# mfkiwl/erlangnetwork-gnsslib-sdr

Measured on AMD Instinct MI355X. Metric: correlations/sec (1 ms coh) + x real-time, 32-SV L1CA @16.368 Msps, higher is better.
Workload: dtype int8 samples x int8 carrier LUT -> int32 accumulators (exact); NCOs: the reference's fp64 running sums, bit for bit; 1 GPU; BASELINE configs[2]: 32-SV GPS L1CA tracking, 5-tap E/P/L correlators (CORRN=2, CORRD=3), 1 ms coherent, 16.368 Msps int8 IQ, per GPU; channels_per_gpu=32, epochs_per_launch=1000, taps=5, loop=open (frequencies held per launch); see closed_loop (--full), if_broadcast=none (1 GPU)

## Files before the change

erlangnetwork-gnsslib-sdr_amd/csrc/gnsscorr_nco.h:

```cpp
#pragma once

#include <math.h>
#include <stdint.h>
#include <string.h>
#include <type_traits>

#if defined(__HIPCC__)
#define GC_HD __host__ __device__ inline
#define GC_HDM __host__ __device__
#define GC_HD_NOINLINE __host__ __device__ __attribute__((noinline))
#else
#define GC_HD static inline
#define GC_HDM
#define GC_HD_NOINLINE static
#endif
#if defined(__clang__)
#define GC_FP_STRICT _Pragma("clang fp contract(off)")
#else
#define GC_FP_STRICT
#endif

#if defined(__HIP_DEVICE_COMPILE__)
#define GC_DDIV(a, b) __ddiv_rn((a), (b))
#else
// ... 1488 lines not shown
    GC_FP_STRICT
    if (C.ex0 == GC_NO_TABLE || n < 1) return false;
    double x = gc_div_y(remcarr * GC_NCO_CDIV, GC_NCO_DPI, P.ydpi);
    if (!gc_one_binade_walk(x, C.s, n, &x)) return false;
    bool held;
    const double p = gc_prem_checked(x, kprem, &held);
    if (!held) return false;
    *remcarr_out = p;
    return true;
}

#define GC_REC_TAG(c)    ((c) & 3)
#define GC_REC_NMATCH    (1 << 2)
#define GC_REC_WALK      (1 << 3)
#define GC_REC_P0(c)     (((c) >> 4) & 15)
#define GC_REC_PLAST(c)  (((c) >> 8) & 15)
#define GC_REC_KPREM(c)  (((c) >> 12) & 15)
#define GC_REC_TIE       (1 << 16)
#define GC_REC_ONE       (1 << 17)
#define GC_REC_ROW1      (1 << 18)
struct GcCarRec {
    double lo, hi;
    double dmd[GC_CLAIM_CWIN];
    int ctl;
    int key;
};

GC_HD bool gc_one_binade_consts(int ex, double s, double *d, bool *tie, double *top)
{
    GC_FP_STRICT
    const uint64_t us = gc_d2u(s);
    const int es = gc_expo(s);
    *tie = false;
    if (ex == 0 || ex == 0x7FF || es == 0 || es == 0x7FF) return false;
    const int et = es + 1075 - ex;
    if (et >= 1023 + 51) return false;
    double b = 0.0;
    if (et >= 1023 - 1) {
        const double t = gc_u2d((us & 0x800FFFFFFFFFFFFFull) | ((uint64_t)et << 52));
        b = rint(t);
        *tie = fabs(t - b) == 0.5;
    }
    *d = ldexp(b, ex - 1075);
    *top = gc_u2d(((uint64_t)ex << 52) | 0x000FFFFFFFFFFFFFull);
    return true;
}

GC_HD void gc_car_rec_make(GcCarRec &R, const GcCarClaims &row, int n, int ilo, int ex0, double s, double ydpi)
{
    GC_FP_STRICT
    int tag = row.tag & 3;
    const int p0 = row.i0 - ilo, plast = p0 + row.nseg - 1;
    if (tag == 1 && !(p0 >= 0 && plast >= p0 && plast < GC_CLAIM_CWIN)) tag = 3;
    if ((tag == 1 || tag == 2) && !(row.kprem >= 0 && row.kprem <= GC_CLAIM_PREM)) tag = 3;
    int ctl = tag | ((row.tag & 3) == 1 ? GC_REC_ROW1 : 0);
    ctl |= n == row.nl ? GC_REC_NMATCH : 0;
    ctl |= (n > 0 && n <= (1 << 24)) ? GC_REC_WALK : 0;
    R.lo = row.lo;
    R.hi = row.hi;
    R.key = 0;
    for (int p = 0; p < GC_CLAIM_CWIN; p++) R.dmd[p] = 0.0;
    if (tag == 1) {
        ctl |= (p0 << 4) | (plast << 8) | (row.kprem << 12);
        for (int p = 0; p < GC_CLAIM_CWIN; p++) R.dmd[p] = (double)row.dm[p];
    } else if (tag == 2) {
        ctl |= row.kprem << 12;
        const double xlo = gc_div_y(row.lo * GC_NCO_CDIV, GC_NCO_DPI, ydpi);
        const double xhi = gc_div_y(row.hi * GC_NCO_CDIV, GC_NCO_DPI, ydpi);
        const int klo = (int)(gc_d2u(xlo) >> 52), khi = (int)(gc_d2u(xhi) >> 52);
        double d, top;
        bool tie;
        if (ex0 != GC_NO_TABLE && klo == khi && (klo >> 11) == (int)(gc_d2u(s) >> 63) &&
            gc_one_binade_consts(klo & 0x7FF, s, &d, &tie, &top)) {
            ctl |= GC_REC_ONE | (tie ? GC_REC_TIE : 0);
            R.key = klo;
            R.dmd[0] = d;
            R.dmd[1] = top;
            R.dmd[2] = (double)n;
        }
    }
    R.ctl = ctl;
}

GC_HD bool gc_carrier_rec_step_one(double ydpi, double remcarr, int key, bool tie, double d, double top, double nd, int kprem,
                                   double *remcarr_out)
{
    GC_FP_STRICT
    const double x = gc_div_y(remcarr * GC_NCO_CDIV, GC_NCO_DPI, ydpi);
    const uint64_t ux = gc_d2u(x);
    if ((int)(ux >> 52) != key) return false;
    if (tie && (ux & 1)) return false;
    const double y = fma(nd, d, x);
    if (!(fabs(y) <= top)) return false;
    bool held;
    const double p = gc_prem_checked(y, kprem, &held);
    if (!held) return false;
    *remcarr_out = p;
    return true;
}

struct GcCodeScanRow {
    long long Yhat, K;
    double r1;
    int valid, pad;
};

GC_HD double gc_code_scan_head(double remcode, double smaxci, double dlen, bool *neg, int *ecs)
{
    GC_FP_STRICT
    const double cs = remcode - smaxci;
    *neg = cs < 0.0;
    *ecs = gc_expo(cs);
    return cs + dlen;
}

GC_HD double gc_code_scan_u(double dlen) { return gc_u2d((uint64_t)(gc_expo(gc_u2d(gc_d2u(dlen) - 1)) - 52) << 52); }
GC_HD double gc_code_scan_invu(double dlen) { return gc_u2d((uint64_t)(2046 - (gc_expo(gc_u2d(gc_d2u(dlen) - 1)) - 52)) << 52); }

GC_HD void gc_code_scan_row(GcCodeScanRow &R, const GcCodePlan &P, double lo, double hi, double r1lo, double r1hi)
{
    GC_FP_STRICT
    R.Yhat = R.K = 0;
    R.r1 = r1lo;
    R.valid = R.pad = 0;
    if (!P.ok || P.it >= P.itop) return;
    const int etop = gc_expo(P.limtop);
    bool n0, n1, n2, n3;
    int e0, e1, e2, e3;
    const double y0 = gc_code_scan_head(lo, P.smaxci, P.dlen, &n0, &e0), y1 = gc_code_scan_head(hi, P.smaxci, P.dlen, &n1, &e1);
    const double z0 = gc_code_scan_head(r1lo, P.smaxci, P.dlen, &n2, &e2), z1 = gc_code_scan_head(r1hi, P.smaxci, P.dlen, &n3, &e3);
    if (!(n0 && n1 && n2 && n3) || e0 != e1 || e2 != e3) return;
    if (gc_expo(y0) != etop || gc_expo(y1) != etop || gc_expo(z0) != etop || gc_expo(z1) != etop) return;
    if (!(y0 < P.dlen && y1 < P.dlen && z0 < P.dlen && z1 < P.dlen)) return;
    const double invu = gc_code_scan_invu(P.dlen);
    const double k0 = (z0 - y0) * invu, k1 = (z1 - y1) * invu;
    if (!(k0 == k1) || !(fabs(k0) < 4503599627370496.0) || floor(k0) != k0) return;
    R.Yhat = (long long)(y0 * invu);
    R.K = (long long)k0;
    R.valid = 1;
}

GC_HD double gc_code_scan_next(double r1, long long Yhat, long long Y, double u)
{
    GC_FP_STRICT
    return r1 + (double)(Y - Yhat) * u;
}
```

erlangnetwork-gnsslib-sdr_amd/csrc/gnsscorr_plan.hip:

```cpp
#include <cstdlib>
#include <cstddef>
#include <hip/hip_runtime.h>

#include "gnsscorr_internal.h"

namespace {


#define GC_SPEC_WC  9.313225746154785e-10
#define GC_SPEC_WK  9.313225746154785e-10

struct SpecChan {
    GcCodePlan PC;
    GcCarPlan PK;
    GcCarStepC CK;
    double ci, spc, ps, dlen;
    int clen, smax;
    int tmax;
    bool ok;
};

__device__ __forceinline__ void spec_chan_init(SpecChan &C, const GcChan &c, const GcTrkState &s, bool with_prem)
{
    C.ci = __dmul_rn(c.ti, s.codefreq);
// ... 102 lines not shown
    srow.r1 = 0.0;
    srow.valid = srow.pad = 0;
    if (C.ok) {
        double r0, g0;
        int nhat;
        gc_spec_start(s.remcode, s.remcarr, C.ci, C.spc, C.ps, C.dlen, e, &r0, &g0, &nhat);
        const double rt = r0 + sumc, gt = g0 + sumk;
        int ncode = 0;
        bool bracketed = false;
#pragma unroll 1
        for (int att = 0; att < 2 && !bracketed; att++) {
            const double w = att == 0 ? GC_SPEC_WC : GC_SPEC_WC * 0.00390625;
            const double lo = rt - w, hi = rt + w;
            const int nlo = gc_period_nsamp(C.dlen, lo, C.spc), nhi = gc_period_nsamp(C.dlen, hi, C.spc);
            if (!(nlo == nhi && nlo > 0 && nlo <= (1 << 24))) continue;
            double flo = 0.0, fhi = 0.0;
            const bool side = (lo - C.PC.smaxci < 0.0) == (hi - C.PC.smaxci < 0.0);
            const bool oklo = gc_code_claims<true>(C.PC, lo, nlo + 2 * C.smax, cc, &flo);
            const bool okhi = oklo && gc_code_claims<false>(C.PC, hi, nlo + 2 * C.smax, cc, &fhi);
            const bool tailfits = nlo + 2 * C.smax - cc.jsum <= C.tmax;
            if (side && oklo && okhi && tailfits) {
                bracketed = true;
                ncode = nlo;
                cc.tag = 1;
                cc.n = nlo;
                cc.lo = lo;
                cc.hi = hi;
                gc_code_scan_row(srow, C.PC, lo, hi, flo, fhi);
            }
        }
        if (!bracketed) {
            ncode = gc_period_nsamp(C.dlen, rt, C.spc);
            cc.tag = 0;
            if (ncode > 0 && ncode <= (1 << 24)) {
                double dummy;
                cc.tag = (gc_code_claims<true>(C.PC, rt, ncode + 2 * C.smax, cc, &dummy) && ncode + 2 * C.smax - cc.jsum <= C.tmax) ? 3 : 0;
            }
            cc.n = ncode;
            cc.lo = cc.hi = rt;
        }
        const int nk = ncode;
        if (nk > 0 && nk <= (1 << 24)) {
            bool kbr = false;
            int tag = 0;
#pragma unroll 1
            for (int att = 0; att < 2 && !kbr; att++) {
                const double w = fmax(GC_SPEC_WK, fabs(gt) * 1.4551915228366852e-11) * (att == 0 ? 1.0 : 0.00390625);
                const double klo = gt - w, khi = gt + w;
                double dummy;
                bool ok = gc_carrier_claims_step<true>(C.PK, C.CK, klo, nk, ck, &dummy);
                tag = ck.tag;
                ok = ok && gc_carrier_claims_step<false, true>(C.PK, C.CK, khi, nk, ck, &dummy);
                if (ok) {
                    kbr = true;
                    ck.tag = tag;
                    ck.lo = klo;
                    ck.hi = khi;
                }
            }
            if (!kbr) {
                double dummy;
                const bool ok = gc_carrier_claims_step<true>(C.PK, C.CK, gt, nk, ck, &dummy);
                ck.tag = ok ? (ck.tag == 2 ? 2 : 3) : 0;
                ck.lo = ck.hi = gt;
            }
            ck.nl = nk;
        }
    }
    const size_t row = (size_t)ch * nepoch + eb;
    int4 *rc = reinterpret_cast<int4 *>(claims_code) + row * (GC_CLAIM_ROW / 4);
    int4 *rk = reinterpret_cast<int4 *>(claims_car) + row * (GC_CLAIM_ROW / 4);
    const int4 *pc4 = reinterpret_cast<const int4 *>(&cc), *pk4 = reinterpret_cast<const int4 *>(&ck);
#pragma unroll
    for (int q = 0; q < GC_CLAIM_ROW / 4; q++) {
        rc[q] = pc4[q];
        rk[q] = pk4[q];
    }
    scan[row] = srow;
}

__device__ unsigned long long gc_plan_stats[8];
#define GC_PLAN_REC_CH 64
__device__ unsigned long long gc_plan_rec[2 * GC_PLAN_REC_CH];
__device__ unsigned long long gc_plan_scan[GC_PLAN_REC_CH];

__host__ __device__ inline int plan2_class(double ti, double codefreq, int clen, int smax)
{
    const double ci = ti * codefreq;
    if (!(ci > 0.0) || !gc_fast_has_table(ci)) return -1;
    const int itop = gc_expo(gc_u2d(gc_d2u((double)clen) - 1)) - (gc_expo(ci) + 2);
    if (itop < 7 || itop > 12) return -1;
    if (smax + 1 > GC_CLAIM_TAIL2) return -1;
    return (itop - 7) * 3 + gc_tail_class(smax);
}

#define GC_PLAN_MAXE 4096
__device__ __attribute__((noinline)) void trk_plan_body(const GcChan *__restrict__ chan,
                                                        const GcTrkState *__restrict__ state_in,
                                                        GcTrkState *__restrict__ state_out,
                                                        GcTrkPlan *__restrict__ plan, int nch, int nepoch)
{
    __shared__ int nsh[GC_PLAN_MAXE];
    __shared__ int prog;
    const int ch = blockIdx.x, lane = threadIdx.x & 63, wave = threadIdx.x >> 6;
    if (ch >= nch) return;
    __builtin_amdgcn_s_setprio(3);
    const bool split = nepoch <= GC_PLAN_MAXE;
    if (threadIdx.x == 0) prog = 0;
    __syncthreads();
    if (!split && wave == 1) return;
    const GcChan c = chan[ch];
    GcTrkState s = state_in[ch];
    const double ci = __dmul_rn(c.ti, s.codefreq);
    const double spc = __ddiv_rn(s.codefreq, c.f_sf);
    const double ps = gc_carrier_ps(s.carrfreq, c.ti);
    const double dlen = (double)c.clen;
    const bool code_ok = ci > 0.0 && ci < dlen;
    GcTrkPlan *out = plan + (size_t)ch * nepoch;
    GcNoEmit ne;
    GcFillLanes fill{lane};
    const bool do_code = wave == 0, do_car = wave == 1 || !split;
    GcCodePlan PC;
    GcCarPlan PK;
    if (do_code) gc_code_plan_init(PC, ci, c.clen, c.smax);
    if (do_car) gc_car_plan_init(PK, ps);
    const double yspc = gc_period_yspc(spc);
    unsigned tally[6] = {0, 0, 0, 0, 0, 0};
    for (int e = 0; e < nepoch; e++) {
        int n;
        if (do_code) {
            n = gc_period_nsamp(dlen, s.remcode, spc, yspc);
            if (lane == 0) {
                out[e].buffloc = s.buffloc;
                out[e].coff = s.remcode;
                out[e].carrfreq = s.carrfreq;
                out[e].codefreq = s.codefreq;
                out[e].n = n;
                out[e].pad = 0;
            }
            if (split) {
                if (lane == 0) nsh[e] = n;
                __threadfence_block();
                if (lane == 0) __hip_atomic_store(&prog, e + 1, __ATOMIC_RELEASE, __HIP_MEMORY_SCOPE_WORKGROUP);
            }
        } else {
            while (__hip_atomic_load(&prog, __ATOMIC_ACQUIRE, __HIP_MEMORY_SCOPE_WORKGROUP) <= e) __builtin_amdgcn_s_sleep(1);
            n = nsh[e];
        }
        const bool walk = n > 0 && n <= (1 << 24);
        if (do_car) {
            if (lane == 0) out[e].phi0 = s.remcarr;
            if (walk) {
                int tier;
                s.remcarr = gc_carrier_period_any(PK, s.remcarr, n, fill, ne, &tier);
                if (tier == GC_TIER_PERIOD) tally[4]++;
                else tally[5]++;
            }
        }
        if (do_code) {
            if (walk && code_ok) {
                int tier;
                s.remcode = gc_code_period_any(PC, s.remcode, n + 2 * c.smax, fill, ne, &tier);
                if (tier == GC_TIER_PERIOD) tally[1]++;
                else tally[2]++;
            }
            s.buffloc += (uint64_t)(int64_t)n;
// ... 30 lines not shown
    GcCarPlan pkfull;
};
__shared__ __attribute__((aligned(16))) Plan4Shared g_plan4;

__device__ __forceinline__ int plan2_uni(int v) { return __builtin_amdgcn_readfirstlane(v); }
template <class T>
__device__ __forceinline__ T *plan2_uni(T *p)
{
    const uint64_t u = (uint64_t)p;
    const unsigned lo = (unsigned)__builtin_amdgcn_readfirstlane((int)(unsigned)u);
    const unsigned hi = (unsigned)__builtin_amdgcn_readfirstlane((int)(unsigned)(u >> 32));
    return (T *)(((uint64_t)hi << 32) | lo);
}
__device__ __forceinline__ double plan2_uni(double x)
{
    const uint64_t u = gc_d2u(x);
    const unsigned lo = (unsigned)__builtin_amdgcn_readfirstlane((int)(unsigned)u);
    const unsigned hi = (unsigned)__builtin_amdgcn_readfirstlane((int)(unsigned)(u >> 32));
    return gc_u2d(((uint64_t)hi << 32) | lo);
}

#define GC_CONST __attribute__((address_space(4)))
typedef int gc_v4i __attribute__((ext_vector_type(4)));
__device__ __forceinline__ GcCodeClaims plan4_code_row(const GC_CONST gc_v4i *r)
{
    const gc_v4i v0 = r[0], v1 = r[1], v2 = r[2], v3 = r[3], v4 = r[4], v5 = r[5];
    GcCodeClaims c;
    c.tag = v0.x; c.i0 = v0.y; c.q = v0.z; c.nl = v0.w;
    c.jsum = v1.x; c.dm[0] = v1.y; c.dm[1] = v1.z; c.dm[2] = v1.w;
    c.dm[3] = v2.x; c.dm[4] = v2.y; c.dm[5] = v2.z; c.dm[6] = v2.w;
    c.dm[7] = v3.x; c.dm[8] = v3.y; c.dm[9] = v3.z; c.dm[10] = v3.w;
    c.dm[11] = v4.x; c.dm[12] = v4.y; c.n = v4.z; c.pad = 0;
    c.lo = gc_u2d(((uint64_t)(unsigned)v5.y << 32) | (unsigned)v5.x);
    c.hi = gc_u2d(((uint64_t)(unsigned)v5.w << 32) | (unsigned)v5.z);
    return c;
}
template <class RowPtr>
__device__ __forceinline__ GcCarClaims plan4_car_row(RowPtr r)
{
    const gc_v4i v0 = r[0], v1 = r[1], v2 = r[2], v3 = r[3], v5 = r[5];
    GcCarClaims c;
    c.tag = v0.x; c.nl = v0.y; c.i0 = v0.z; c.nseg = v0.w;
    c.kprem = v1.x; c.dm[0] = v1.y; c.dm[1] = v1.z; c.dm[2] = v1.w;
    c.dm[3] = v2.x; c.dm[4] = v2.y; c.dm[5] = v2.z; c.dm[6] = v2.w;
    c.dm[7] = v3.x; c.dm[8] = v3.y; c.dm[9] = v3.z; c.dm[10] = v3.w;
    c.dm[11] = 0; c.dm[12] = 0; c.pad[0] = 0; c.pad[1] = 0;
    c.lo = gc_u2d(((uint64_t)(unsigned)v5.y << 32) | (unsigned)v5.x);
    c.hi = gc_u2d(((uint64_t)(unsigned)v5.w << 32) | (unsigned)v5.z);
    return c;
}
static_assert(GC_CLAIM_CWIN <= 11, "plan4_car_row reads dm[0..10]");
static_assert(sizeof(GcCodeClaims) == GC_CLAIM_ROW * 4 && sizeof(GcCarClaims) == GC_CLAIM_ROW * 4, "claims rows are GC_CLAIM_ROW ints");
static_assert(offsetof(GcCodeClaims, dm) == 20 && offsetof(GcCarClaims, dm) == 20, "claims layout");
static_assert(offsetof(GcCodeClaims, n) == 72 && offsetof(GcCodeClaims, lo) == 80 && offsetof(GcCarClaims, lo) == 80, "claims layout");
static_assert(GC_CLAIM_ROW == 24, "plan4_*_row read six int4 per row");

__device__ __attribute__((noinline)) int plan2_code_slow(double ci_, int clen_, int smax_, double remcode_, int n_, int lane, double *out)
{
    const double ci = plan2_uni(ci_), remcode = plan2_uni(remcode_);
    const int clen = plan2_uni(clen_), smax = plan2_uni(smax_), n = plan2_uni(n_);
    GcCodePlan PC;
    gc_code_plan_init(PC, ci, clen, smax);
    GcFillLanes fill{lane};
    GcNoEmit ne;
    int tier;
    *out = gc_code_period_any(PC, remcode, n + 2 * smax, fill, ne, &tier);
    return tier == GC_TIER_PERIOD ? 1 : 2;
}

__device__ __attribute__((noinline)) int plan2_car_slow(double remcarr_, int n_, int lane, double *out)
{
    const double remcarr = plan2_uni(remcarr_);
    const int n = plan2_uni(n_);
    const GcCarPlan &PK = g_plan4.pkfull;
    GcFillLanes fill{lane};
    GcNoEmit ne;
    int tier;
    *out = gc_carrier_period_any(PK, remcarr, n, fill, ne, &tier);
    return tier == GC_TIER_PERIOD ? 1 : 2;
}

#ifdef GC_PLAN_PROF
__device__ unsigned long long gc_plan_prof[64 * 16];
#define GC_PP_DECL unsigned long long pp_[7] = {0, 0, 0, 0, 0, 0, 0}
#define GC_PP_T0(v) const unsigned long long v = __builtin_readcyclecounter()
#define GC_PP_ADD(k, v) pp_[k] += __builtin_readcyclecounter() - (v)
#define GC_PP_INC(k) pp_[k] += 1
#define GC_PP_ADDN(k, n) pp_[k] += (n)
#define GC_PP_OUT(which) do { if (lane == 0 && blockIdx.x < 64) for (int k_ = 0; k_ < 7; k_++) atomicAdd(&gc_plan_prof[blockIdx.x * 16 + (which) * 8 + k_], pp_[k_]); } while (0)
#else
#define GC_PP_DECL do { } while (0)
#define GC_PP_T0(v) do { } while (0)
#define GC_PP_ADD(k, v) do { } while (0)
#define GC_PP_INC(k) do { } while (0)
#define GC_PP_ADDN(k, n) do { } while (0)
#define GC_PP_OUT(which) do { } while (0)
#endif
struct Plan4Job {
    const int4 *claims_code, *claims_car;
    const GcCodeScanRow *scan;
    GcTrkPlan *out;
    GcTrkState *state_out;
    GcTrkState s;
    int nepoch, nblk, verify;
};

__device__ __forceinline__ Plan4Job plan4_job(const Plan4Job *J_)
{
    Plan4Job J = *plan2_uni(J_);
    J.claims_code = plan2_uni(J.claims_code);
    J.claims_car = plan2_uni(J.claims_car);
    J.scan = plan2_uni(J.scan);
    J.out = plan2_uni(J.out);
    J.state_out = plan2_uni(J.state_out);
    J.nepoch = plan2_uni(J.nepoch);
    J.nblk = plan2_uni(J.nblk);
    J.verify = plan2_uni(J.verify);
    return J;
}

__device__ __forceinline__ int plan4_nb(const Plan4Job &J, int b)
{
    const int left = J.nepoch - b * GC_P4_BLK;
    return left < GC_P4_BLK ? left : GC_P4_BLK;
}

#define GC_GLOBAL __attribute__((address_space(1)))
__device__ __forceinline__ void plan4_publish(int v)
{
    asm volatile("" ::: "memory");
    __hip_atomic_store(&g_plan4.prog, v, __ATOMIC_RELAXED, __HIP_MEMORY_SCOPE_WORKGROUP);
}
__device__ __forceinline__ int plan4_progress()
{
    const int v = __hip_atomic_load(&g_plan4.prog, __ATOMIC_RELAXED, __HIP_MEMORY_SCOPE_WORKGROUP);
    asm volatile("" ::: "memory");
    return v;
}
template <int ITOP, int TMAX>
__device__ __attribute__((noinline)) int plan4_code_other(double ci_, int clen_, int smax_, double remcode_, int n_, int lane, const GcCodeClaims *cl_, double *out)
{
    const GcCodeClaims *clp = plan2_uni(cl_);
    if (plan2_uni(clp->tag) == 1 || plan2_uni(clp->tag) == 3) {
        const double ci = plan2_uni(ci_), remcode = plan2_uni(remcode_);
        const int clen = plan2_uni(clen_), smax = plan2_uni(smax_), n = plan2_uni(n_);
        GcCodePlan PC;
        gc_code_plan_init(PC, ci, clen, smax, false);
        GcCodeStepC<ITOP> SC;
        gc_code_stepc_init(SC, PC);
        GcCodeClaims c2 = *clp;
        c2.tag = 1;
        double rc;
        if (gc_code_claims_step<ITOP, TMAX, false, true>(PC, SC, remcode, n + 2 * smax, c2, &rc)) { *out = rc; return 0; }
    }
    return plan2_code_slow(ci_, clen_, smax_, remcode_, n_, lane, out);
}

__device__ __forceinline__ int plan4_scopy(int x)
{
    int c;
    asm volatile("s_mov_b32 %0, %1" : "=s"(c) : "s"(x));
    return c;
}
__device__ __forceinline__ bool plan4_bcopy(bool x) { return __builtin_amdgcn_readfirstlane(x ? 1 : 0) != 0; }

__device__ __forceinline__ long long plan4_wscan(long long v, int lane)
// ... 255 lines not shown
        const int n = plan2_uni(n_), nsamp = plan2_uni(nsamp_);
        GcCarPlan PK;
        gc_car_plan_init(PK, ps, false, false);
        GcCarStepC CK;
        gc_car_stepc_init(CK, PK, nsamp + 16);
        GcCarClaims c2 = *clp;
        c2.tag = tag == 2 ? 2 : 1;
        double rp;
        if (gc_carrier_claims_step<false, true>(PK, CK, remcarr, n, c2, &rp)) { *out = rp; return 0; }
    }
    return plan2_car_slow(remcarr_, n_, lane, out);
}

__device__ __attribute__((noinline)) void plan4_car_cert_wave(double ps_, const Plan4Job *J_, int lane)
{
    const double ps = plan2_uni(ps_);
    const Plan4Job J = plan4_job(J_);
    GcCarPlan PK;
    gc_car_plan_init(PK, ps);
    GcFillLanes fill{lane};
    GcNoEmit ne;
    unsigned tally1 = 0, tally2 = 0;
    GC_GLOBAL GcTrkPlan *out = (GC_GLOBAL GcTrkPlan *)J.out;
    double remcarr = J.s.remcarr;
    int seen = 0;
    for (int b = 0; b < J.nblk; b++) {
        const int nb = plan4_nb(J, b), e0 = b * GC_P4_BLK;
        for (int i = 0; i < nb; i++) {
            while (seen <= e0 + i) {
                seen = plan2_uni(plan4_progress());
                if (seen <= e0 + i) __builtin_amdgcn_s_sleep(1);
            }
            const int n = plan2_uni(g_plan4.nsh[e0 + i]);
            if (lane == 0) g_plan4.vstart[1][i] = remcarr;
            if (n > 0 && n <= (1 << 24)) {
                int tier;
                remcarr = gc_carrier_period_any(PK, remcarr, n, fill, ne, &tier);
                tally1 += tier == GC_TIER_PERIOD ? 1 : 0;
                tally2 += tier == GC_TIER_PERIOD ? 0 : 1;
            }
        }
        if (lane < nb) out[e0 + lane].phi0 = g_plan4.vstart[1][lane];
    }
    if (lane == 0) {
        ((GC_GLOBAL GcTrkState *)J.state_out)->remcarr = remcarr;
        if (tally1) atomicAdd(&gc_plan_stats[4], (unsigned long long)tally1);
        if (tally2) atomicAdd(&gc_plan_stats[5], (unsigned long long)tally2);
    }
}

__device__ __attribute__((noinline)) int plan4_car_one(double s_, int ex0_, double remcarr_, int n_, int ctl_, int key_, double d_, double top_,
                                                       double nd_, int verify_, double *out)
{
    const int verify = plan2_uni(verify_);
    const double s = plan2_uni(s_), remcarr = plan2_uni(remcarr_), d = plan2_uni(d_), top = plan2_uni(top_), nd = plan2_uni(nd_);
    const int ex0 = plan2_uni(ex0_), n = plan2_uni(n_), ctl = plan2_uni(ctl_), key = plan2_uni(key_);
    GcCarPlan P;
    P.ydpi = 1.0 / GC_NCO_DPI;
    GcCarStepC C;
    C.s = s;
    C.ex0 = ex0;
    double r = remcarr, r2 = remcarr;
    const bool done = gc_carrier_value_step_one(P, C, remcarr, n, GC_REC_KPREM(ctl), &r);
    int bad = 0;
    if (verify && (ctl & GC_REC_ONE)) {
        const bool done2 = gc_carrier_rec_step_one(P.ydpi, remcarr, key, (ctl & GC_REC_TIE) != 0, d, top, nd, GC_REC_KPREM(ctl), &r2);
        bad = (done2 && (!done || gc_d2u(r2) != gc_d2u(r))) ? 2 : 0;
    }
    if (done) *out = r;
    return (done ? 1 : 0) | bad;
}

__device__ __forceinline__ void plan4_rec_load(GcCarRec &R, int i)
{
    const GcCarRec &r = g_plan4.rec[i];
    R.lo = r.lo;
    R.hi = r.hi;
#pragma unroll
    for (int p = 0; p < GC_CLAIM_CWIN; p++) R.dmd[p] = r.dmd[p];
    R.ctl = r.ctl;
    R.key = r.key;
}

struct Plan4CarRun {
    double remcarr, phi;
    unsigned recwin, recone;
    unsigned tally0, tally1, tally2, miss, mism, slow;
    unsigned long long slowclk;
};

#ifdef GC_PLAN_PROF
#define GC_PP_SLOW0(v) const unsigned long long v = __builtin_readcyclecounter()
#define GC_PP_SLOW1(S, v) (S).slowclk += __builtin_readcyclecounter() - (v)
#else
#define GC_PP_SLOW0(v) do { } while (0)
#define GC_PP_SLOW1(S, v) do { } while (0)
#endif

__device__ __forceinline__ void plan4_car_period(Plan4CarRun &S, const GcCarRec &R, const GcCarPlan &PK, const GcCarStepC &CK, double ps, int nsamp,
                                                 const Plan4Job &J, int e, int i, int lane)
{
    const int ctl = plan2_uni(R.ctl);
    const int tag = GC_REC_TAG(ctl);
    const double remcarr = S.remcarr;
    const bool inside_u = plan4_bcopy(remcarr >= R.lo && remcarr <= R.hi) && (ctl & (3 | GC_REC_NMATCH)) == (1 | GC_REC_NMATCH);
    S.phi = lane == i ? remcarr : S.phi;
    if (!(ctl & GC_REC_WALK)) return;
    double rp = remcarr;
    bool done = false;
    if (inside_u && !J.verify) {
        rp = gc_carrier_value_step(PK, CK, remcarr, GC_REC_P0(ctl), GC_REC_PLAST(ctl), GC_REC_KPREM(ctl), R.dmd);
        done = true;
        S.recwin++;
    } else if (tag == 2) {
        if ((ctl & GC_REC_ONE) && !J.verify) {
            double r2 = remcarr;
            done = plan4_bcopy(gc_carrier_rec_step_one(PK.ydpi, remcarr, plan2_uni(R.key), (ctl & GC_REC_TIE) != 0, R.dmd[0], R.dmd[1], R.dmd[2],
                                                       GC_REC_KPREM(ctl), &r2));
            rp = done ? r2 : rp;
            S.recone += done ? 1 : 0;
        }
        if (!done) {
            double r1;
            const int n = plan2_uni(g_plan4.nsh[e]);
            GC_PP_SLOW0(pone_);
            const int how = plan4_car_one(CK.s, CK.ex0, remcarr, n, ctl, R.key, R.dmd[0], R.dmd[1], R.dmd[2], J.verify, &r1);
            GC_PP_SLOW1(S, pone_);
            done = (how & 1) != 0;
            S.slow++;
            S.tally0 += done ? 1 : 0;
            S.mism += (how & 2) ? 1 : 0;
            if (done) rp = r1;
        }
    }
    if (!done) {
        double rs;
        const int n = plan2_uni(g_plan4.nsh[e]);
        GC_PP_SLOW0(pother_);
        const int how = plan4_car_other(ps, nsamp, remcarr, n, lane, reinterpret_cast<const GcCarClaims *>(J.claims_car) + e, &rs);
        GC_PP_SLOW1(S, pother_);
        S.slow++;
        S.tally0 += how == 0 ? 1 : 0;
        S.tally1 += how == 1 ? 1 : 0;
        S.tally2 += how == 2 ? 1 : 0;
        S.mism += (inside_u && how != 0) ? 1 : 0;
        S.miss += (!inside_u && (ctl & GC_REC_ROW1)) ? 1 : 0;
        rp = rs;
    }
    S.remcarr = rp;
}

__device__ __attribute__((noinline)) void plan4_car_wave(double ps_, int nsamp_, const Plan4Job *J_, int lane)
{
    const int nsamp = plan2_uni(nsamp_);
    const double ps = plan2_uni(ps_);
    const Plan4Job J = plan4_job(J_);
    {
        const int nlook = J.nepoch < 16 ? J.nepoch : 16;
        int none = 0;
        for (int e = 0; e < nlook; e++)
            none += ((const GC_CONST int *)J.claims_car)[(size_t)e * GC_CLAIM_ROW] == 0 ? 1 : 0;
        if (none == nlook && nlook >= 8) {
            plan4_car_cert_wave(ps, J_, lane);
            return;
        }
    }
    {
        GcCarPlan full;
        gc_car_plan_init(full, ps);
        if (lane == 0) g_plan4.pkfull = full;
    }
    GcCarPlan PK;
    gc_car_plan_init(PK, ps, false, false);
    GcCarStepC CK;
    gc_car_stepc_init(CK, PK, nsamp + 16);
    const int ilo = plan2_uni(CK.ilo), ex0 = plan2_uni(CK.ex0);
    GC_GLOBAL GcTrkPlan *out = (GC_GLOBAL GcTrkPlan *)J.out;
    Plan4CarRun S;
    S.remcarr = J.s.remcarr;
    S.phi = 0.0;
    S.recwin = S.recone = S.tally0 = S.tally1 = S.tally2 = S.miss = S.mism = S.slow = 0;
    S.slowclk = 0;
    int seen = 0;
    GC_PP_DECL;
    GC_PP_T0(ptot_);
    for (int b = 0; b < J.nblk; b++) {
        const int nb = plan4_nb(J, b), e0 = b * GC_P4_BLK;
        GC_PP_T0(ptop_);
        const int el = e0 + (lane < nb ? lane : nb - 1);
        const GcCarClaims row = plan4_car_row((const GC_GLOBAL gc_v4i *)J.claims_car + (size_t)el * (GC_CLAIM_ROW / 4));
        if (seen < e0 + nb) {
            GC_PP_T0(pn_);
            while (seen < e0 + nb) {
                seen = plan2_uni(plan4_progress());
                if (seen < e0 + nb) __builtin_amdgcn_s_sleep(1);
            }
            GC_PP_ADD(3, pn_);
        }
        {
            GcCarRec mine;
            gc_car_rec_make(mine, row, g_plan4.nsh[el], ilo, ex0, CK.s, PK.ydpi);
            if (lane < nb) g_plan4.rec[lane] = mine;
        }
        asm volatile("" ::: "memory");
        __builtin_amdgcn_wave_barrier();
        GC_PP_ADD(5, ptop_);
        GC_PP_T0(pstep_);
        GcCarRec A, B;
        plan4_rec_load(A, 0);
        for (int i = 0; i < nb; i += 2) {
            plan4_rec_load(B, i + 1 < nb ? i + 1 : i);
            __builtin_amdgcn_sched_barrier(0);
            plan4_car_period(S, A, PK, CK, ps, nsamp, J, e0 + i, i, lane);
            if (i + 1 >= nb) break;
            plan4_rec_load(A, i + 2 < nb ? i + 2 : i + 1);
            __builtin_amdgcn_sched_barrier(0);
            plan4_car_period(S, B, PK, CK, ps, nsamp, J, e0 + i + 1, i + 1, lane);
        }
        GC_PP_ADD(6, pstep_);
        if (lane < nb) out[e0 + lane].phi0 = S.phi;
    }
    GC_PP_ADD(0, ptot_);
    GC_PP_ADDN(1, S.slowclk);
    GC_PP_ADDN(4, S.slow);
    GC_PP_OUT(1);
    if (lane == 0) {
        ((GC_GLOBAL GcTrkState *)J.state_out)->remcarr = S.remcarr;
        S.tally0 += S.recwin + S.recone;
        if (blockIdx.x < GC_PLAN_REC_CH) {
            if (S.recwin) atomicAdd(&gc_plan_rec[blockIdx.x * 2], (unsigned long long)S.recwin);
            if (S.recone) atomicAdd(&gc_plan_rec[blockIdx.x * 2 + 1], (unsigned long long)S.recone);
        }
        if (S.tally0) atomicAdd(&gc_plan_stats[3], (unsigned long long)S.tally0);
        if (S.tally1) atomicAdd(&gc_plan_stats[4], (unsigned long long)S.tally1);
        if (S.tally2) atomicAdd(&gc_plan_stats[5], (unsigned long long)S.tally2);
        if (S.mism) atomicAdd(&gc_plan_stats[6], (unsigned long long)S.mism);
        if (S.miss) atomicAdd(&gc_plan_stats[7], (unsigned long long)S.miss);
    }
}

template <int ITOP>
__device__ __forceinline__ void plan4_code_dispatch(int tcls, double ci, double spc, int clen, int smax, const Plan4Job *J, int lane)
{
    if (tcls == 0) plan4_code_wave<ITOP, gc_tail_max(0)>(ci, spc, clen, smax, J, lane);
    else if (tcls == 1) plan4_code_wave<ITOP, gc_tail_max(1)>(ci, spc, clen, smax, J, lane);
    else plan4_code_wave<ITOP, gc_tail_max(2)>(ci, spc, clen, smax, J, lane);
}

__global__ __launch_bounds__(128) void trk_plan4_kernel(const GcChan *__restrict__ chan, const GcTrkState *__restrict__ state_in,
                                                        GcTrkState *__restrict__ state_out, GcTrkPlan *__restrict__ plan,
                                                        int nch, int nepoch, const int *__restrict__ claims_code,
                                                        const int *__restrict__ claims_car, const GcCodeScanRow *__restrict__ scan, int verify)
{
    const int ch = blockIdx.x, tid = threadIdx.x, lane = tid & 63, wave = tid >> 6;
    if (ch >= nch) return;
    const GcChan c = chan[ch];
    const GcTrkState s = state_in[ch];
    const double ci = __dmul_rn(c.ti, s.codefreq), spc = __ddiv_rn(s.codefreq, c.f_sf), ps = gc_carrier_ps(s.carrfreq, c.ti);
    const int cls = plan2_class(c.ti, s.codefreq, c.clen, c.smax);
    if (cls < 0 || !(ci > 0.0 && ci < (double)c.clen)) {
        trk_plan_body(chan, state_in, state_out, plan, nch, nepoch);
        return;
    }
    const int itop = cls / 3 + 7, tcls = cls % 3;
    constexpr int RW4 = GC_CLAIM_ROW / 4;
    Plan4Job J;
    J.claims_code = reinterpret_cast<const int4 *>(claims_code) + (size_t)ch * nepoch * RW4;
    J.claims_car = reinterpret_cast<const int4 *>(claims_car) + (size_t)ch * nepoch * RW4;
    J.scan = scan ? scan + (size_t)ch * nepoch : nullptr;
    J.out = plan + (size_t)ch * nepoch;
    J.state_out = state_out + ch;
    J.s = s;
    J.nepoch = nepoch;
    J.nblk = (nepoch + GC_P4_BLK - 1) / GC_P4_BLK;
    J.verify = verify;
    if (tid == 0) g_plan4.prog = 0;
    __syncthreads();
    __builtin_amdgcn_s_setprio(3);
    if (wave == 0) {
        gc_with_itop(itop, [&](auto IT) { plan4_code_dispatch<decltype(IT)::value>(tcls, ci, spc, c.clen, c.smax, &J, lane); return true; });
    } else {
        plan4_car_wave(ps, c.nsamp, &J, lane);
    }
}


}


#ifdef GC_PLAN_PROF
extern "C" int gnsscorr_debug_plan_prof(unsigned long long *dst)
{
    if (hipMemcpyFromSymbol(dst, HIP_SYMBOL(gc_plan_prof), sizeof(unsigned long long) * 64 * 16) != hipSuccess) return -1;
    return 0;
}
#endif

extern "C" int gnsscorr_debug_plan_stats(unsigned long long *dst, int reset)
{
    if (hipMemcpyFromSymbol(dst, HIP_SYMBOL(gc_plan_stats), sizeof(unsigned long long) * 8) != hipSuccess) return -1;
    if (reset) {
        unsigned long long z[8] = {0, 0, 0, 0, 0, 0, 0, 0};
        if (hipMemcpyToSymbol(HIP_SYMBOL(gc_plan_stats), z, sizeof(z)) != hipSuccess) return -1;
    }
    return 0;
}

extern "C" int gnsscorr_debug_plan_rec(unsigned long long *dst, int reset)
{
    if (hipMemcpyFromSymbol(dst, HIP_SYMBOL(gc_plan_rec), sizeof(unsigned long long) * 2 * GC_PLAN_REC_CH) != hipSuccess) return -1;
    if (reset) {
        unsigned long long z[2 * GC_PLAN_REC_CH] = {0};
        if (hipMemcpyToSymbol(HIP_SYMBOL(gc_plan_rec), z, sizeof(z)) != hipSuccess) return -1;
    }
    return 0;
}

extern "C" int gnsscorr_debug_plan_scan(unsigned long long *dst, int reset)
{
    if (hipMemcpyFromSymbol(dst, HIP_SYMBOL(gc_plan_scan), sizeof(unsigned long long) * GC_PLAN_REC_CH) != hipSuccess) return -1;
    if (reset) {
        unsigned long long z[GC_PLAN_REC_CH] = {0};
        if (hipMemcpyToSymbol(HIP_SYMBOL(gc_plan_scan), z, sizeof(z)) != hipSuccess) return -1;
    }
    return 0;
}

static bool trk_nospec()
{
    static const bool nospec = getenv("GNSSCORR_TRK_NOSPEC") != nullptr;
    return nospec;
}

size_t gc_trk_spec_ints(size_t units) { return units * (2 * GC_CLAIM_ROW + 8 + 8); }
static_assert(sizeof(GcCodeScanRow) == 32 && ((2 * GC_CLAIM_ROW + 8) * 4) % 32 == 0, "scan rows lie 32-byte aligned behind the deviations");
static GcCodeScanRow *trk_scan_rows(int *claims, size_t units) { return reinterpret_cast<GcCodeScanRow *>(claims + units * (2 * GC_CLAIM_ROW + 8)); }

int gc_launch_trk_spec(hipStream_t st, const GcChan *chan, const GcTrkState *state_in, int nch, int nepoch, int *claims,
                       int e_off)
{
    if (!claims || trk_nospec() || nepoch > GC_PLAN_MAXE || e_off < 0 || e_off > nepoch) return 0;
    const size_t units = (size_t)nch * nepoch;
    const int T = e_off + nepoch;
    double *devc = reinterpret_cast<double *>(claims + 2 * units * GC_CLAIM_ROW), *devk = devc + 2 * units;
    hipLaunchKernelGGL(trk_specdev_kernel, dim3((nch * T + 63) / 64), dim3(64), 0, st, chan, state_in, devc, devk, nch, T);
    GC_HIP(hipGetLastError());
    const int nchunk = (nepoch + GC_SPEC_CHUNK - 1) / GC_SPEC_CHUNK;
    hipLaunchKernelGGL(trk_spec_kernel, dim3(nch * nchunk), dim3(GC_SPEC_CHUNK), 0, st, chan, state_in, devc, devk, claims,
                       claims + units * GC_CLAIM_ROW, trk_scan_rows(claims, units), nch, nepoch, e_off);
    GC_HIP(hipGetLastError());
    return 0;
}

int gc_launch_trk_plan(hipStream_t st, const GcChan *chan, const GcTrkState *state_in, GcTrkState *state_out,
                       GcTrkPlan *plan, int nch, int nepoch, int *claims)
{
    static const int verify = getenv("GNSSCORR_PLAN_VERIFY") ? atoi(getenv("GNSSCORR_PLAN_VERIFY")) : 0;
    const bool batch = claims && !trk_nospec() && nepoch <= GC_PLAN_MAXE;
    if (batch)
        hipLaunchKernelGGL(trk_plan4_kernel, dim3(nch), dim3(128), 0, st, chan, state_in, state_out, plan, nch, nepoch,
                           claims, claims + (size_t)nch * nepoch * GC_CLAIM_ROW,
                           (const GcCodeScanRow *)trk_scan_rows(claims, (size_t)nch * nepoch), verify);
    else
        hipLaunchKernelGGL(trk_plan_kernel, dim3(nch), dim3(128), 0, st, chan, state_in, state_out, plan, nch, nepoch);
    GC_HIP(hipGetLastError());
    return 0;
}
```

erlangnetwork-gnsslib-sdr_amd/csrc/gnsscorr_trk.hip:

```cpp
#include <cstdlib>
#include <type_traits>


#include "gnsscorr_ctx.h"
#include "gnsscorr_ps.h"

namespace {


#define GC_EXP_LANES 64
struct ExpCarTable {
    int *k0;
    GcCarSeg *seg;
    int cap, n, overflow, prevk;
    bool lastzero, bad;
    __device__ void operator()(int k, double x, double d, int )
    {
        const GcCarSeg s = gc_carseg_make(x, d);
        const bool zero = s.fx == 0 && s.dfx == 0;
        if (n > 0 && zero && lastzero) return;
        if (n >= cap) { overflow = 1; return; }
        bad = bad || (n == 0 ? k != 0 : !(prevk < k));
        k0[n] = k;
        seg[n] = s;
// ... 726 lines not shown
    GC_RESERVE(ctx, o.dcorrI, units * ctx->ntap);
    GC_RESERVE(ctx, o.dcorrQ, units * ctx->ntap);
    GC_RESERVE(ctx, o.nsamp, units);
    GC_RESERVE(ctx, o.dsumI, (size_t)ctx->nch * ctx->ntap);
    GC_RESERVE(ctx, o.dsumQ, (size_t)ctx->nch * ctx->ntap);
    for (GcDevBuf<int> *c : {&o.dnco_overflow, &o.dring_viol}) {
        if (*c) continue;
        GC_RESERVE(ctx, *c, 1);
        GC_HIP(hipMemsetAsync(*c, 0, sizeof(int), ctx->stream));
    }
    o.units = units;
    return GNSSCORR_OK;
}

static int ensure_batch_buffers(gnsscorr_ctx *ctx, int nepoch)
{
    GcBatch &b = ctx->batch;
    const size_t units = (size_t)ctx->nch * nepoch;
    if (units <= b.units) return GNSSCORR_OK;
    GC_TRY(gc_drain(ctx));
    b.ahead_valid = false;
    b.spec_ahead_valid = false;
    b.units = 0;
    b.nseg = 1;
    for (int i = 0; i < ctx->nch; i++) {
        const int s = gc_trk_nseg(ctx->hchan[i].dtype, ctx->max_n);
        if (s > b.nseg) b.nseg = s;
    }
    for (GcPlanSlot &s : b.slot) {
        GC_RESERVE(ctx, s.plan, units);
        GC_RESERVE(ctx, s.partial, units * b.nseg * 2 * ctx->ntap);
        GC_RESERVE(ctx, s.unit, units);
        GC_RESERVE(ctx, s.rounds, units * b.nseg * GC_MAXR);
        GC_RESERVE(ctx, s.segs, units);
        GC_RESERVE(ctx, s.etab, units * GC_EDGTAB);
    }
    for (int i = 0; i < 2; i++) GC_RESERVE(ctx, b.dspec2[i], gc_trk_spec_ints(units));
    GC_RESERVE(ctx, b.dfinish, (size_t)ctx->nch * GC_FINISH_SCRATCH);
    GC_HIP(hipMemsetAsync(b.dfinish, 0, sizeof(unsigned long long) * ctx->nch * GC_FINISH_SCRATCH, ctx->stream));
    b.units = units;
    return GNSSCORR_OK;
}

static int plan_into(gnsscorr_ctx *ctx, int s, int nepoch, hipEvent_t gate)
{
    GcBatch &b = ctx->batch;
    GcPlanSlot &sl = b.slot[s];
    hipStream_t ps = ctx->stream_plan;
    const GcTrkState *sin = ctx->state.cur();
    int buf;
    if (b.spec_pending) GC_HIP(hipStreamWaitEvent(ps, ctx->ev_spec, 0));
    if (b.spec_ahead_valid && !ctx->state.touched && b.spec_ahead_nepoch == nepoch && b.spec_ahead_state == (const void *)sin) {
        buf = b.spec_ahead_buf;
    } else {
        buf = 0;
        GC_HIP(hipStreamWaitEvent(ps, ctx->ev_tab[s], 0));
        GcTimed t(ctx, "trk_spec", ps);
        GC_TRY(gc_launch_trk_spec(ps, ctx->dchan, sin, ctx->nch, nepoch, b.dspec2[buf], 0));
    }
    b.spec_ahead_valid = false;
    b.spec_pending = false;
    b.spec_last_buf = buf;
    b.spec_last_units = ctx->nch * nepoch;
    GC_HIP(hipStreamWaitEvent(ctx->stream_discover, gate, 0));
    {
        GcTimed t(ctx, "trk_spec", ctx->stream_discover);
        GC_TRY(gc_launch_trk_spec(ctx->stream_discover, ctx->dchan, sin, ctx->nch, nepoch, b.dspec2[buf ^ 1], nepoch));
    }
    GC_HIP(hipStreamWaitEvent(ctx->stream_discover, ctx->ev_tab[s ^ 1], 0));
    GC_HIP(hipEventRecord(ctx->ev_spec, ctx->stream_discover));
    b.spec_pending = true;
    b.spec_ahead_valid = true;
    b.spec_ahead_buf = buf ^ 1;
    b.spec_ahead_nepoch = nepoch;
    b.spec_ahead_state = (const void *)ctx->state.next();
    {
        GcTimed t(ctx, "trk_plan", ps);
        GC_TRY(gc_launch_trk_plan(ps, ctx->dchan, sin, ctx->state.next(), sl.plan, ctx->nch, nepoch, b.dspec2[buf]));
    }
    GC_HIP(hipEventRecord(ctx->ev_plan[s], ps));
    return GNSSCORR_OK;
}

static int correlate_slot(gnsscorr_ctx *ctx, int s, int nepoch, const uint64_t wr[2])
{
    GcBatch &b = ctx->batch;
    GcPlanSlot &sl = b.slot[s];
    hipStream_t ts = ctx->stream_tables;
    GC_HIP(hipStreamWaitEvent(ts, ctx->ev_plan[s], 0));
    GC_HIP(hipStreamWaitEvent(ts, ctx->ev_corr[s], 0));
    GC_HIP(hipStreamWaitEvent(ts, ctx->ev_corr[s ^ 1], 0));
    {
        GcTimed t(ctx, "trk_expand", ts);
        GC_TRY(gc_launch_trk_expand(ts, ctx->dchan, sl.plan, sl.unit, sl.segs, ctx->out.nsamp, ctx->nch, nepoch,
                                    sl.rounds, b.nseg, ctx->max_n, ctx->out.dnco_overflow));
    }
    GC_TRY(launch_trk_ringcheck(ts, ctx->dchan, sl.plan, (const int8_t *)ctx->ring[0].mem, wr[0], wr[1], ctx->nch,
                                nepoch, ctx->out.dring_viol));
    {
        GcTimed t(ctx, "trk_edges", ts);
        GC_TRY(launch_trk_edges(ts, ctx->dchan, sl.unit, sl.segs, sl.etab, ctx->nch, nepoch));
    }
    GC_HIP(hipEventRecord(ctx->ev_tab[s], ts));
    GC_HIP(hipStreamWaitEvent(ctx->stream, ctx->ev_tab[s], 0));
    for (int dtype = 1; dtype <= 2; dtype++) {
        if (!ctx->have_dtype[dtype]) continue;
        GcTimed t(ctx, "trk_corr");
        GC_TRY(gc_launch_trk_corr(ctx->stream, ctx->dchan, sl.unit, sl.segs, sl.rounds, sl.partial, ctx->nch, nepoch, b.nseg,
                                  ctx->ntap, dtype, ctx->ntap, ctx->max_n, ctx->smax_max, sl.etab));
    }
    GC_HIP(hipEventRecord(ctx->ev_corr[s], ctx->stream));
    return GNSSCORR_OK;
}

static int finish_slot(gnsscorr_ctx *ctx, int s, int nepoch)
{
    GcBatch &b = ctx->batch;
    GcTrkOut &o = ctx->out;
    GcTimed t(ctx, "trk_finish");
    GC_TRY(gc_launch_trk_finish(ctx->stream, b.slot[s].partial, o.dcorrI, o.dcorrQ, o.dsumI, o.dsumQ, b.dfinish, ctx->nch,
                                nepoch, b.nseg, ctx->ntap));
    o.fin_pending = true;
    return GNSSCORR_OK;
}

extern "C" int gnsscorr_trk_run(gnsscorr_ctx *ctx, int nepoch)
{
    if (!ctx || nepoch <= 0) return gc_fail(GNSSCORR_EINVAL, "trk_run: nepoch %d", nepoch);
    if (!ctx->nch) return gc_fail(GNSSCORR_ESTATE, "trk_run: no channels set");
    GC_HIP(hipSetDevice(ctx->device));
    GC_TRY(gc_ensure_trk_outputs(ctx, nepoch));
    GC_TRY(ensure_batch_buffers(ctx, nepoch));
    uint64_t wr[2];
    GC_TRY(gc_ring_positions(ctx, wr));
    GcBatch &b = ctx->batch;
    hipStream_t ps = ctx->stream_plan;
    const int cur = b.plan_slot;
    if (!(b.ahead_valid && b.ahead_nepoch == nepoch)) {
        if (b.ahead_valid) {
            GC_HIP(hipStreamSynchronize(ps));
            b.ahead_valid = false;
        }
        GC_HIP(hipEventRecord(ctx->ev_used[cur], ctx->stream));
        GC_HIP(hipStreamWaitEvent(ps, ctx->ev_used[cur], 0));
        GC_TRY(plan_into(ctx, cur, nepoch, ctx->ev_used[cur]));
    }
    GC_TRY(correlate_slot(ctx, cur, nepoch, wr));
    b.ahead_valid = false;
    ctx->state.commit();
    b.plan_slot ^= 1;
    if (!ctx->state.touched) {
        GC_TRY(plan_into(ctx, b.plan_slot, nepoch, ctx->ev_plan[cur]));
        b.ahead_valid = true;
        b.ahead_nepoch = nepoch;
    }
    ctx->state.touched = false;
    GC_TRY(finish_slot(ctx, cur, nepoch));
    ctx->out.last_nepoch = nepoch;
    ctx->loop.last_nper = 0;
    return GNSSCORR_OK;
}

int gc_nco_check(gnsscorr_ctx *ctx)
{
    GcTrkOut &o = ctx->out;
    int n = 0, v = 0;
    GC_HIP(hipMemcpy(&v, o.dring_viol, sizeof(int), hipMemcpyDeviceToHost));
    if (v) {
        GC_HIP(hipMemset(o.dring_viol, 0, sizeof(int)));
        return gc_fail(GNSSCORR_ESTATE, "tracking: %d (channel, period) units lay outside what the IF ring holds "
                       "(beyond the write position, or overwritten since): their sums are not the stream's", v);
    }
    GC_HIP(hipMemcpy(&n, o.dnco_overflow, sizeof(int), hipMemcpyDeviceToHost));
    if (!n) return GNSSCORR_OK;
// ... 75 lines not shown
```

Before: 312.3 million correlations/s.

## Batch eligible carrier-NCO record steps into wave-uniform runs with vectorized validation

In the plan4 carrier pass, consecutive epochs whose records are single-binade walk records with a shared step constant are advanced as a run. A scalar loop computes each step's phase, then one ballot checks every step's validity conditions in parallel. Any rejected step falls back to the per-epoch period path, so the per-record serial checks and branching are meant to be paid once per run instead of once per epoch. The change also adds run and reject counters and profiling, and gates the tables-stream wait on the previous slot's correlation behind a macro whose default keeps the wait. The exactness of the fp64 running sums depends on the new multiply-based remainder matching the old checked remainder path.

```diff
diff --git a/erlangnetwork-gnsslib-sdr_amd/csrc/gnsscorr_nco.h b/erlangnetwork-gnsslib-sdr_amd/csrc/gnsscorr_nco.h
--- a/erlangnetwork-gnsslib-sdr_amd/csrc/gnsscorr_nco.h
+++ b/erlangnetwork-gnsslib-sdr_amd/csrc/gnsscorr_nco.h
@@ -1594,10 +1594,43 @@
     R.ctl = ctl;
 }
 
+GC_HD double gc_carrier_run_value(double ydpi, double remcarr, double d, double nd)
+{
+    GC_FP_STRICT
+    const double x = gc_div_y(remcarr * GC_NCO_CDIV, GC_NCO_DPI, ydpi);
+    const double y = fma(nd, d, x);
+    return y * GC_NCO_DPI * (1.0 / GC_NCO_CDIV);
+}
+
+GC_HD bool gc_carrier_run_eligible(int ctl)
+{
+    return (ctl & (GC_REC_ONE | GC_REC_WALK)) == (GC_REC_ONE | GC_REC_WALK) && GC_REC_KPREM(ctl) == 0;
+}
+
+GC_HD bool gc_carrier_run_holds(double ydpi, double remcarr, int ctl, int key, double d, double top, double nd)
+{
+    GC_FP_STRICT
+    const double x = gc_div_y(remcarr * GC_NCO_CDIV, GC_NCO_DPI, ydpi);
+    const uint64_t ux = gc_d2u(x);
+    const double y = fma(nd, d, x);
+    const double p = y * GC_NCO_DPI * (1.0 / GC_NCO_CDIV);
+    const bool inkey = (int)(ux >> 52) == key;
+    const bool odd_tie = ((ctl & GC_REC_TIE) != 0) & ((ux & 1) != 0);
+    const bool intop = fabs(y) <= top;
+    const bool held = (p < 1.0e300) & !(p > GC_NCO_DPI);
+    return gc_carrier_run_eligible(ctl) & inkey & !odd_tie & intop & held;
+}
+
 GC_HD bool gc_carrier_rec_step_one(double ydpi, double remcarr, int key, bool tie, double d, double top, double nd, int kprem,
                                    double *remcarr_out)
 {
     GC_FP_STRICT
+    if (kprem == 0) {
+        const int ctl = GC_REC_ONE | GC_REC_WALK | (tie ? GC_REC_TIE : 0);
+        if (!gc_carrier_run_holds(ydpi, remcarr, ctl, key, d, top, nd)) return false;
+        *remcarr_out = gc_carrier_run_value(ydpi, remcarr, d, nd);
+        return true;
+    }
     const double x = gc_div_y(remcarr * GC_NCO_CDIV, GC_NCO_DPI, ydpi);
     const uint64_t ux = gc_d2u(x);
     if ((int)(ux >> 52) != key) return false;
diff --git a/erlangnetwork-gnsslib-sdr_amd/csrc/gnsscorr_plan.hip b/erlangnetwork-gnsslib-sdr_amd/csrc/gnsscorr_plan.hip
--- a/erlangnetwork-gnsslib-sdr_amd/csrc/gnsscorr_plan.hip
+++ b/erlangnetwork-gnsslib-sdr_amd/csrc/gnsscorr_plan.hip
@@ -208,6 +208,7 @@
 __device__ unsigned long long gc_plan_stats[8];
 #define GC_PLAN_REC_CH 64
 __device__ unsigned long long gc_plan_rec[2 * GC_PLAN_REC_CH];
+__device__ unsigned long long gc_plan_run[4 * GC_PLAN_REC_CH];
 __device__ unsigned long long gc_plan_scan[GC_PLAN_REC_CH];
 
 __host__ __device__ inline int plan2_class(double ti, double codefreq, int clen, int smax)
@@ -404,6 +405,7 @@
 
 #ifdef GC_PLAN_PROF
 __device__ unsigned long long gc_plan_prof[64 * 16];
+__device__ unsigned long long gc_plan_prof_run[64 * 2];
 #define GC_PP_DECL unsigned long long pp_[7] = {0, 0, 0, 0, 0, 0, 0}
 #define GC_PP_T0(v) const unsigned long long v = __builtin_readcyclecounter()
 #define GC_PP_ADD(k, v) pp_[k] += __builtin_readcyclecounter() - (v)
@@ -825,11 +827,21 @@
     R.key = r.key;
 }
 
+__device__ __forceinline__ double plan4_readlane_d(double x, int l)
+{
+    const uint64_t u = gc_d2u(x);
+    const unsigned lo = (unsigned)__builtin_amdgcn_readlane((int)(unsigned)u, l);
+    const unsigned hi = (unsigned)__builtin_amdgcn_readlane((int)(unsigned)(u >> 32), l);
+    return gc_u2d(((uint64_t)hi << 32) | lo);
+}
+
 struct Plan4CarRun {
     double remcarr, phi;
     unsigned recwin, recone;
     unsigned tally0, tally1, tally2, miss, mism, slow;
+    unsigned runs, racc, rej, rejchk;
     unsigned long long slowclk;
+    unsigned long long runclk, chkclk;
 };
 
 #ifdef GC_PLAN_PROF
@@ -923,8 +935,10 @@
     S.remcarr = J.s.remcarr;
     S.phi = 0.0;
     S.recwin = S.recone = S.tally0 = S.tally1 = S.tally2 = S.miss = S.mism = S.slow = 0;
-    S.slowclk = 0;
+    S.runs = S.racc = S.rej = S.rejchk = 0;
+    S.slowclk = S.runclk = S.chkclk = 0;
     int seen = 0;
+    bool inrun = false;
     GC_PP_DECL;
     GC_PP_T0(ptot_);
     for (int b = 0; b < J.nblk; b++) {
@@ -940,25 +954,82 @@
             }
             GC_PP_ADD(3, pn_);
         }
+        int mctl, mkey;
+        double md, mtop, mnd;
         {
             GcCarRec mine;
             gc_car_rec_make(mine, row, g_plan4.nsh[el], ilo, ex0, CK.s, PK.ydpi);
             if (lane < nb) g_plan4.rec[lane] = mine;
-        }
+            mctl = mine.ctl;
+            mkey = mine.key;
+            md = mine.dmd[0];
+            mtop = mine.dmd[1];
+            mnd = mine.dmd[2];
+        }
+        const unsigned long long em = __ballot(lane < nb && !J.verify && gc_carrier_run_eligible(mctl));
+        const unsigned long long sm = __ballot(gc_d2u(md) == gc_d2u(__shfl_up(md, 1, 64)));
         asm volatile("" ::: "memory");
         __builtin_amdgcn_wave_barrier();
         GC_PP_ADD(5, ptop_);
         GC_PP_T0(pstep_);
         GcCarRec A, B;
-        plan4_rec_load(A, 0);
-        for (int i = 0; i < nb; i += 2) {
-            plan4_rec_load(B, i + 1 < nb ? i + 1 : i);
-            __builtin_amdgcn_sched_barrier(0);
-            plan4_car_period(S, A, PK, CK, ps, nsamp, J, e0 + i, i, lane);
-            if (i + 1 >= nb) break;
-            plan4_rec_load(A, i + 2 < nb ? i + 2 : i + 1);
-            __builtin_amdgcn_sched_barrier(0);
-            plan4_car_period(S, B, PK, CK, ps, nsamp, J, e0 + i + 1, i + 1, lane);
+        if (em != 0) {
+            int i = 0;
+            while (i < nb) {
+                if ((em >> i) & 1ull) {
+                    const unsigned long long cont = ~((em >> i) & ((sm >> i) | 1ull));
+                    const int m = cont ? (int)__builtin_ctzll(cont) : 64;
+                    GC_PP_SLOW0(prun_);
+                    const double d = plan4_readlane_d(md, i);
+                    double r = S.remcarr;
+                    for (int k = 0; k < m; k++) {
+                        S.phi = lane == i + k ? r : S.phi;
+                        r = gc_carrier_run_value(PK.ydpi, r, d, plan4_readlane_d(mnd, i + k));
+                    }
+#ifdef GC_PLAN_PROF
+                    S.runclk += __builtin_readcyclecounter() - prun_;
+#endif
+                    GC_PP_SLOW0(pchk_);
+                    const bool in = lane >= i && lane < i + m;
+                    const bool ok = gc_carrier_run_holds(PK.ydpi, S.phi, mctl, mkey, md, mtop, mnd);
+                    const unsigned long long bad = __ballot(in && !ok);
+                    const int f = bad ? (int)__builtin_ctzll(bad) : i + m;
+                    const bool rejected = f < i + m;
+                    if (rejected) r = plan4_readlane_d(S.phi, f);
+                    S.remcarr = r;
+                    S.runs++;
+                    S.racc += (unsigned)(f - i);
+                    S.recone += (unsigned)(f - i);
+                    inrun = f > i || inrun;
+                    S.rejchk += rejected ? 1 : 0;
+                    S.rej += rejected ? 1 : 0;
+                    inrun = rejected ? false : inrun;
+                    i = f;
+#ifdef GC_PLAN_PROF
+                    S.chkclk += __builtin_readcyclecounter() - pchk_;
+#endif
+                    if (!rejected) continue;
+                } else {
+                    S.rej += inrun ? 1 : 0;
+                    inrun = false;
+                }
+                plan4_rec_load(A, i);
+                plan4_car_period(S, A, PK, CK, ps, nsamp, J, e0 + i, i, lane);
+                i++;
+            }
+        } else {
+            S.rej += inrun ? 1 : 0;
+            inrun = false;
+            plan4_rec_load(A, 0);
+            for (int i = 0; i < nb; i += 2) {
+                plan4_rec_load(B, i + 1 < nb ? i + 1 : i);
+                __builtin_amdgcn_sched_barrier(0);
+                plan4_car_period(S, A, PK, CK, ps, nsamp, J, e0 + i, i, lane);
+                if (i + 1 >= nb) break;
+                plan4_rec_load(A, i + 2 < nb ? i + 2 : i + 1);
+                __builtin_amdgcn_sched_barrier(0);
+                plan4_car_period(S, B, PK, CK, ps, nsamp, J, e0 + i + 1, i + 1, lane);
+            }
         }
         GC_PP_ADD(6, pstep_);
         if (lane < nb) out[e0 + lane].phi0 = S.phi;
@@ -967,12 +1038,24 @@
     GC_PP_ADDN(1, S.slowclk);
     GC_PP_ADDN(4, S.slow);
     GC_PP_OUT(1);
+#ifdef GC_PLAN_PROF
+    if (lane == 0 && blockIdx.x < 64) {
+        atomicAdd(&gc_plan_prof_run[blockIdx.x * 2], S.runclk);
+        atomicAdd(&gc_plan_prof_run[blockIdx.x * 2 + 1], S.chkclk);
+    }
+#endif
     if (lane == 0) {
         ((GC_GLOBAL GcTrkState *)J.state_out)->remcarr = S.remcarr;
         S.tally0 += S.recwin + S.recone;
         if (blockIdx.x < GC_PLAN_REC_CH) {
             if (S.recwin) atomicAdd(&gc_plan_rec[blockIdx.x * 2], (unsigned long long)S.recwin);
             if (S.recone) atomicAdd(&gc_plan_rec[blockIdx.x * 2 + 1], (unsigned long long)S.recone);
+            if (S.runs) {
+                atomicAdd(&gc_plan_run[blockIdx.x * 4], (unsigned long long)S.runs);
+                atomicAdd(&gc_plan_run[blockIdx.x * 4 + 1], (unsigned long long)S.racc);
+            }
+            if (S.rej) atomicAdd(&gc_plan_run[blockIdx.x * 4 + 2], (unsigned long long)S.rej);
+            if (S.rejchk) atomicAdd(&gc_plan_run[blockIdx.x * 4 + 3], (unsigned long long)S.rejchk);
         }
         if (S.tally0) atomicAdd(&gc_plan_stats[3], (unsigned long long)S.tally0);
         if (S.tally1) atomicAdd(&gc_plan_stats[4], (unsigned long long)S.tally1);
@@ -1039,6 +1122,14 @@
 }
 #endif
 
+#ifdef GC_PLAN_PROF
+extern "C" int gnsscorr_debug_plan_prof_run(unsigned long long *dst)
+{
+    if (hipMemcpyFromSymbol(dst, HIP_SYMBOL(gc_plan_prof_run), sizeof(unsigned long long) * 64 * 2) != hipSuccess) return -1;
+    return 0;
+}
+#endif
+
 extern "C" int gnsscorr_debug_plan_stats(unsigned long long *dst, int reset)
 {
     if (hipMemcpyFromSymbol(dst, HIP_SYMBOL(gc_plan_stats), sizeof(unsigned long long) * 8) != hipSuccess) return -1;
@@ -1055,6 +1146,16 @@
     if (reset) {
         unsigned long long z[2 * GC_PLAN_REC_CH] = {0};
         if (hipMemcpyToSymbol(HIP_SYMBOL(gc_plan_rec), z, sizeof(z)) != hipSuccess) return -1;
+    }
+    return 0;
+}
+
+extern "C" int gnsscorr_debug_plan_run(unsigned long long *dst, int reset)
+{
+    if (hipMemcpyFromSymbol(dst, HIP_SYMBOL(gc_plan_run), sizeof(unsigned long long) * 4 * GC_PLAN_REC_CH) != hipSuccess) return -1;
+    if (reset) {
+        unsigned long long z[4 * GC_PLAN_REC_CH] = {0};
+        if (hipMemcpyToSymbol(HIP_SYMBOL(gc_plan_run), z, sizeof(z)) != hipSuccess) return -1;
     }
     return 0;
 }
diff --git a/erlangnetwork-gnsslib-sdr_amd/csrc/gnsscorr_trk.hip b/erlangnetwork-gnsslib-sdr_amd/csrc/gnsscorr_trk.hip
--- a/erlangnetwork-gnsslib-sdr_amd/csrc/gnsscorr_trk.hip
+++ b/erlangnetwork-gnsslib-sdr_amd/csrc/gnsscorr_trk.hip
@@ -832,6 +832,9 @@
     return GNSSCORR_OK;
 }
 
+#ifndef GC_TRK_TABLES_WAIT_PREV
+#define GC_TRK_TABLES_WAIT_PREV 1
+#endif
 static int correlate_slot(gnsscorr_ctx *ctx, int s, int nepoch, const uint64_t wr[2])
 {
     GcBatch &b = ctx->batch;
@@ -839,7 +842,9 @@
     hipStream_t ts = ctx->stream_tables;
     GC_HIP(hipStreamWaitEvent(ts, ctx->ev_plan[s], 0));
     GC_HIP(hipStreamWaitEvent(ts, ctx->ev_corr[s], 0));
+#if GC_TRK_TABLES_WAIT_PREV
     GC_HIP(hipStreamWaitEvent(ts, ctx->ev_corr[s ^ 1], 0));
+#endif
     {
         GcTimed t(ctx, "trk_expand", ts);
         GC_TRY(gc_launch_trk_expand(ts, ctx->dchan, sl.plan, sl.unit, sl.segs, ctx->out.nsamp, ctx->nch, nepoch,
```

Measured after the change: 314.7 million correlations/s, median of 6. No clear change (+0.8%).
